# dfm/emcee

Measured on NVIDIA H100. Metric: walker-steps/sec (nwalkers x iters / s), higher is better.
Workload: dtype f64

## Files before the change

emcee_b200/csrc/dense_dmma.cu:

```cuda
#include <math.h>

#include "engine.cuh"
#include "tma.cuh"

namespace eb {

namespace {

constexpr int DMMA_CONSUMERS = 8;
constexpr int DMMA_THREADS = 64 * DMMA_CONSUMERS;
constexpr int NI = 2;
constexpr int DMMA_PRODUCER_REGS = 64;
constexpr int DMMA_CONSUMER_REGS = 192;
static_assert((DMMA_THREADS / 2) * (DMMA_PRODUCER_REGS + DMMA_CONSUMER_REGS) <= 65536, "register file of one SM");
__host__ __device__ constexpr bool dmma_rebalance(int KB, bool HAS_MEAN, bool BOUNDED) {
  return !BOUNDED && (KB >= 15 || (HAS_MEAN && KB >= 11));
}

__device__ __forceinline__ void dmma1688(double (&c)[4], double2 a01, double2 a23, double b0, double b1) {
  asm volatile(
      "mma.sync.aligned.m16n8k8.row.col.f64.f64.f64.f64 {%0,%1,%2,%3}, {%4,%5,%6,%7}, {%8,%9}, {%0,%1,%2,%3};"
      : "+d"(c[0]), "+d"(c[1]), "+d"(c[2]), "+d"(c[3])
      : "d"(a01.x), "d"(a01.y), "d"(a23.x), "d"(a23.y), "d"(b0), "d"(b1));
}

__host__ __device__ constexpr int col_pairs(int KB) { return (KB + 1) / 2; }
__host__ __device__ constexpr int factor_dmmas(int KB) { return col_pairs(KB) * (KB - col_pairs(KB) + 1); }
__host__ __device__ constexpr size_t factor_doubles(int KB) { return (size_t)factor_dmmas(KB) * 128; }
__host__ __device__ constexpr int row_stride(int KB) { return 8 * KB + 8; }

struct TileMeta {
  double factor[8];
  double log_u[8];
  double lp_old[8];
  int32_t w[8];
};

template <int KB>
struct SmemLayout {
  static constexpr size_t L_doubles = factor_doubles(KB);
  static constexpr size_t mu_doubles = 8 * KB;
  static constexpr size_t slot_doubles = 2 * 8 * row_stride(KB);
  static constexpr size_t off_mu = L_doubles;
  static constexpr size_t off_slots = off_mu + mu_doubles;
  static constexpr size_t off_meta = off_slots + DMMA_CONSUMERS * slot_doubles;
  static constexpr size_t meta_bytes = sizeof(TileMeta) * 2 * DMMA_CONSUMERS;
  static constexpr size_t off_bars_bytes = off_meta * sizeof(double) + meta_bytes;
  static constexpr int nbars = 1 + 3 * DMMA_CONSUMERS;
  static constexpr size_t off_abort_bytes = off_bars_bytes + nbars * sizeof(uint64_t);
  static constexpr size_t off_inbox_bytes = off_abort_bytes + 16;
  static constexpr size_t total_bytes = off_inbox_bytes + sizeof(int32_t) * 2 * 8 * DMMA_CONSUMERS;
};

template <int KB, bool HAS_MEAN>
__device__ __forceinline__ double tile_sumsq(const double (&q)[2 * KB], const double* sL, const double* sMu, int lane,
                                             int g, int t) {
  constexpr int NP = col_pairs(KB);
  double rs0 = 0.0, rs1 = 0.0;
  const double* aptr = sL + 2 * lane;
#pragma unroll
  for (int m0 = 0; m0 < NP; m0 += NI) {
    double c[NI][4];
#pragma unroll
    for (int n = 0; n < NI; ++n) c[n][0] = c[n][1] = c[n][2] = c[n][3] = 0.0;
#pragma unroll
    for (int j = 2 * m0; j < KB; ++j) {
      double x0 = q[2 * j + 0], x1 = q[2 * j + 1];
      if (HAS_MEAN) {
        const double2 m2 = *reinterpret_cast<const double2*>(sMu + 8 * j + 2 * t);
        x0 -= m2.x;
        x1 -= m2.y;
      }
#pragma unroll
      for (int n = 0; n < NI; ++n) {
        if (m0 + n < NP && j >= 2 * (m0 + n)) {
          const double2 a01 = *reinterpret_cast<const double2*>(aptr);
          const double2 a23 = *reinterpret_cast<const double2*>(aptr + 64);
          dmma1688(c[n], a01, a23, x0, x1);
          aptr += 128;
        }
      }
    }
#pragma unroll
    for (int n = 0; n < NI; ++n) {
      rs0 = fma(c[n][0], c[n][0], rs0);
      rs0 = fma(c[n][2], c[n][2], rs0);
      rs1 = fma(c[n][1], c[n][1], rs1);
      rs1 = fma(c[n][3], c[n][3], rs1);
    }
  }
#pragma unroll
  for (int o = 4; o < 32; o <<= 1) {
    rs0 += __shfl_xor_sync(0xffffffffu, rs0, o);
    rs1 += __shfl_xor_sync(0xffffffffu, rs1, o);
  }
  const double e = __shfl_sync(0xffffffffu, rs0, g >> 1), o = __shfl_sync(0xffffffffu, rs1, g >> 1);
  return (g & 1) ? o : e;
}

__device__ __forceinline__ bool grid_wait(const unsigned long long* counter, unsigned long long target, int* status) {
  const long long t0 = clock64();
  while (*reinterpret_cast<const volatile unsigned long long*>(counter) < target) {
    __nanosleep(32);
    if (clock64() - t0 > 60000000000ll) {
      atomicOr(status, FLAG_COMM_TIMEOUT);
      return false;
    }
  }
  __threadfence();
  return true;
}

__device__ __forceinline__ bool peer_wait(const unsigned* my_flags, int rank, int nranks, unsigned target, int lane,
                                          int* status) {
  bool ok = true;
  if (lane < nranks && lane != rank) {
    const volatile unsigned* f = my_flags + lane;
    const long long t0 = clock64();
    while ((int)(*f - target) < 0) {
      __nanosleep(64);
      if (clock64() - t0 > 60000000000ll) {
        atomicOr(status, FLAG_COMM_TIMEOUT);
        ok = false;
        break;
      }
    }
  }
  __threadfence_system();
  return __all_sync(0xffffffffu, ok);
}

template <int KB, bool HAS_MEAN, bool BOUNDED, bool TIMELINE>
__global__ void __launch_bounds__(DMMA_THREADS, 1)
    half_step_dense_dmma_kernel(const HalfStepArgs a, const HalfDesc d0, const HalfDesc* __restrict__ descs,
                                const int nhalf, unsigned long long* gbar, const unsigned long long gbar_base) {
  constexpr int D = 8 * KB;
  constexpr int RS = row_stride(KB);
  using SL = SmemLayout<KB>;
  extern __shared__ __align__(16) unsigned char smem_raw[];
  double* sL = reinterpret_cast<double*>(smem_raw);
  double* sMu = sL + SL::off_mu;
  double* sSlots = sL + SL::off_slots;
  TileMeta* sMeta = reinterpret_cast<TileMeta*>(sL + SL::off_meta);
  uint64_t* bars = reinterpret_cast<uint64_t*>(smem_raw + SL::off_bars_bytes);
  volatile int* sAbort = reinterpret_cast<volatile int*>(smem_raw + SL::off_abort_bytes);
  volatile int* sPeers = sAbort + 1;
  int32_t* sInbox = reinterpret_cast<int32_t*>(smem_raw + SL::off_inbox_bytes);
  uint64_t* barL = bars;
  uint64_t* barFull = bars + 1;
  uint64_t* barReady = bars + 1 + DMMA_CONSUMERS;
  uint64_t* barFree = bars + 1 + 2 * DMMA_CONSUMERS;

  const int tid = threadIdx.x, lane = tid & 31, warp = tid >> 5;
  const bool is_producer = warp >= DMMA_CONSUMERS;
  const int pair = is_producer ? warp - DMMA_CONSUMERS : warp;
  const int g = lane >> 2, t = lane & 3;

  if (tid == 0) {
    *sAbort = 0;
    *sPeers = 0;
    mbar_init(barL, 1);
    for (int c = 0; c < DMMA_CONSUMERS; ++c) {
      mbar_init(barFull + c, 1);
      mbar_init(barReady + c, 1);
      mbar_init(barFree + c, 1);
    }
    asm volatile("fence.mbarrier_init.release.cluster;" ::: "memory");
  }
  if (HAS_MEAN)
    for (int k = tid; k < D; k += DMMA_THREADS) sMu[k] = a.model.params[k];
  __syncthreads();

  const int tstride = (int)gridDim.x * DMMA_CONSUMERS;
  const int tile0 = (int)blockIdx.x + (int)gridDim.x * pair;
  double* slot = sSlots + (size_t)pair * SL::slot_doubles;
  double* myS = slot + (size_t)g * RS + 2 * t;
  double* myC = myS + 8 * RS;
  TileMeta* meta = sMeta + 2 * pair;
  const bool multi = a.p2p_peer_flags != nullptr;
  unsigned k = 0;

  constexpr bool REBALANCE = dmma_rebalance(KB, HAS_MEAN, BOUNDED);
  if (is_producer) {
    if constexpr (REBALANCE) asm volatile("setmaxnreg.dec.sync.aligned.u32 %0;" ::"n"(DMMA_PRODUCER_REGS));
    const long long t_entry_p = clock64();
    long long* tlp = (TIMELINE && lane == 0)
                         ? a.timeline + ((size_t)blockIdx.x * DMMA_CONSUMERS + pair) * TL_TILES * TL_EVENTS : nullptr;
    const double dm1 = (double)a.D - 1.0;
    const int row = lane & 7;
    struct Prep {
      int32_t w, wp;
      double zz, factor, log_u, lp_old;
      bool valid, remote;
    };
    for (int h = 0; h < nhalf; ++h) {
      const HalfDesc d = (h == 0) ? d0 : descs[h];
      const int32_t* order = a.order + (size_t)d.order_step * a.N;
      const int2 rg = a.range ? a.range[(size_t)d.order_step * MAX_SPLITS + d.split] : make_int2(0, d.a_count);
      const int i_lo = rg.x, i_hi = rg.y;
      const int ntiles = (int)(((int64_t)i_hi - i_lo + 7) >> 3);
      const int64_t Nc = a.N - d.a_count;
      const int32_t* aperm = a.aperm ? a.aperm + (size_t)d.order_step * a.N + d.a_start : nullptr;
      auto prep = [&](int tile, bool with_lp) -> Prep {
        Prep p;
        int i = i_lo + tile * 8 + row;
        p.valid = i < i_hi;
        if (!p.valid) i = i_hi - 1;
        if (aperm) i = __ldg(aperm + i);
        const u32x4 A = draw_words(a.seed, d.step, (uint32_t)d.split, TAG_PROP_A, (uint32_t)i);
        const double tt = __dadd_rn(__dmul_rn(__dsub_rn(a.p0, 1.0), u53(A.x, A.y)), 1.0);
        p.zz = __ddiv_rn(__dmul_rn(tt, tt), a.p0);
        const int64_t r = (int64_t)bounded64(A.z, A.w, (uint64_t)Nc);
        p.w = __ldg(order + d.a_start + i);
        p.wp = __ldg(order + (r < d.a_start ? r : r + d.a_count));
        const u32x4 U = draw_words(a.seed, d.step, (uint32_t)d.split, TAG_ACCEPT, (uint32_t)i);
        p.log_u = log(u53(U.x, U.y));
        p.factor = __dmul_rn(dm1, log(p.zz));
        p.lp_old = with_lp ? a.logp[p.w] : 0.0;
        p.remote = multi && (p.wp / a.rows_per_rank != a.p2p_rank);
        return p;
      };
      auto peers_ready = [&]() -> bool {
        if (!multi || *sPeers > h) return true;
        if (pair == 0) {
          if (!peer_wait(a.p2p_my_flags, a.p2p_rank, a.p2p_nranks, a.p2p_wait + (unsigned)h, lane, a.status)) {
            *sAbort = 1;
            return false;
          }
          __syncwarp();
          if (lane == 0) *sPeers = h + 1;
        } else {
          while (*sPeers <= h) {
            if (*sAbort) return false;
            __nanosleep(64);
          }
        }
        asm volatile("fence.proxy.async;" ::: "memory");
        return true;
      };
      auto request = [&](const Prep& p, int lo, int hi) {
        if (lane >= lo && lane < hi) {
          const bool partner = lane >= 8;
          const int32_t wr = partner ? p.wp : p.w;
          const double* base =
              (partner && a.peer_coords != nullptr) ? a.peer_coords[wr / a.rows_per_rank] : a.coords;
          bulk_g2s(slot + (size_t)(partner ? 8 : 0) * RS + (size_t)row * RS, base + (size_t)wr * D,
                   (unsigned)(D * sizeof(double)), barFull + pair);
        }
      };
      auto publish = [&](const Prep& p, int par) {
        TileMeta* m = meta + par;
        if (lane < 8) {
          m->factor[row] = p.factor;
          m->log_u[row] = p.log_u;
          m->lp_old[row] = p.lp_old;
          m->w[row] = p.valid ? p.w : -1;
        }
      };
      auto issue = [&](Prep& p, int par, bool load_lp) -> bool {
        if (__any_sync(0xffffffffu, p.remote) && !peers_ready()) return false;
        if (lane == 0) mbar_arrive_expect_tx(barFull + pair, 16u * D * (unsigned)sizeof(double));
        __syncwarp();
        request(p, 0, 16);
        if (load_lp) p.lp_old = a.logp[p.w];
        publish(p, par);
        return true;
      };
      Prep cur{}, nxt{};
      const bool early = h == 0 && a.dmma_early_own && tile0 < ntiles;
      if (early) {
        cur = prep(tile0, true);
        if (lane == 0) mbar_arrive_expect_tx(barFull + pair, 16u * D * (unsigned)sizeof(double));
        __syncwarp();
        if (tlp) tlp[6] = clock64() - t_entry_p;
        request(cur, 0, 8);
      } else if (tile0 < ntiles) {
        cur = prep(tile0, false);
      }
      if (h == 0) {
        pdl_wait();
        pdl_launch_dependents();
        if (multi && !a.aperm && !peers_ready()) return;
        if (tile0 < ntiles) {
          if (a.dmma_stagger && pair >= DMMA_CONSUMERS / 2)
            mbar_wait_for(barFull + pair - DMMA_CONSUMERS / 2, 0, multi ? 40000 : 12000);
          if (early) {
            request(cur, 8, 16);
            publish(cur, (int)(k & 1u));
          } else {
            if (tlp) tlp[6] = clock64() - t_entry_p;
            if (!issue(cur, (int)(k & 1u), true)) return;
          }
        }
        if (pair == 0 && !peers_ready()) return;
        if (tile0 + tstride < ntiles) nxt = prep(tile0 + tstride, true);
      } else {
        if (tile0 + tstride < ntiles) nxt = prep(tile0 + tstride, false);
        bool ok = true;
        if (lane == 0) ok = grid_wait(gbar, gbar_base + (unsigned long long)h * gridDim.x, a.status);
        ok = __shfl_sync(0xffffffffu, ok, 0);
        if (!ok) {
          *sAbort = 1;
          return;
        }
        asm volatile("fence.proxy.async;" ::: "memory");
        if (tile0 < ntiles) {
          if (k > 0 && !mbar_wait_abortable(barFree + pair, (k - 1) & 1u, sAbort)) return;
          if (!issue(cur, (int)(k & 1u), true)) return;
        }
      }
      for (int tile = tile0; tile < ntiles; tile += tstride, ++k) {
        const double zz = __shfl_sync(0xffffffffu, cur.zz, g);
        if (!mbar_wait_abortable(barFull + pair, k & 1u, sAbort)) return;
        long long* tlq = (tlp && h == nhalf - 1 && (tile - tile0) / tstride < TL_TILES && lane == 0)
                             ? tlp + ((tile - tile0) / tstride) * TL_EVENTS : nullptr;
        if (tlq) tlq[7] = clock64() - t_entry_p;
        if constexpr (BOUNDED) {
          bool in = true;
#pragma unroll
          for (int j = 0; j < KB; ++j) {
            const double2 s2 = *reinterpret_cast<const double2*>(myS + 8 * j);
            const double2 c2 = *reinterpret_cast<const double2*>(myC + 8 * j);
            double2 q2;
            q2.x = __dsub_rn(c2.x, __dmul_rn(__dsub_rn(c2.x, s2.x), zz));
            q2.y = __dsub_rn(c2.y, __dmul_rn(__dsub_rn(c2.y, s2.y), zz));
            *reinterpret_cast<double2*>(myC + 8 * j) = q2;
            const double2 l2 = __ldg(reinterpret_cast<const double2*>(a.model.lo + 8 * j + 2 * t));
            const double2 h2 = __ldg(reinterpret_cast<const double2*>(a.model.hi + 8 * j + 2 * t));
            in &= (l2.x <= q2.x) & (q2.x <= h2.x) & (l2.y <= q2.y) & (q2.y <= h2.y);
          }
          in &= __shfl_xor_sync(0xffffffffu, in, 1);
          in &= __shfl_xor_sync(0xffffffffu, in, 2);
          if (t == 0) sInbox[(2 * pair + (k & 1u)) * 8 + g] = in ? 1 : 0;
        } else {
#pragma unroll
          for (int j = 0; j < KB; ++j) {
            const double2 s2 = *reinterpret_cast<const double2*>(myS + 8 * j);
            const double2 c2 = *reinterpret_cast<const double2*>(myC + 8 * j);
            double2 q2;
            q2.x = __dsub_rn(c2.x, __dmul_rn(__dsub_rn(c2.x, s2.x), zz));
            q2.y = __dsub_rn(c2.y, __dmul_rn(__dsub_rn(c2.y, s2.y), zz));
            *reinterpret_cast<double2*>(myC + 8 * j) = q2;
          }
        }
        __syncwarp();
        if (lane == 0) mbar_arrive(barReady + pair);
        if (tlq) tlq[8] = clock64() - t_entry_p;
        if (tile + tstride < ntiles) {
          cur = nxt;
          if (!mbar_wait_abortable(barFree + pair, k & 1u, sAbort)) return;
          if (tlq && (tile - tile0) / tstride + 1 < TL_TILES)
            tlq[TL_EVENTS + 6] = clock64() - t_entry_p;
          if (!issue(cur, (int)((k + 1) & 1u), h > 0 && tile == tile0)) return;
          if (tile + 2 * tstride < ntiles) nxt = prep(tile + 2 * tstride, true);
        }
      }
    }
    return;
  }

  if constexpr (REBALANCE) asm volatile("setmaxnreg.inc.sync.aligned.u32 %0;" ::"n"(DMMA_CONSUMER_REGS));
  if (tid == 0) {
    constexpr unsigned bytes = (unsigned)(SL::L_doubles * sizeof(double));
    mbar_arrive_expect_tx(barL, bytes);
    bulk_g2s(sL, a.model.chol, bytes, barL);
  }
  const long long t_entry = clock64();
  long long* tl = TIMELINE ? a.timeline + ((size_t)blockIdx.x * DMMA_CONSUMERS + pair) * TL_TILES * TL_EVENTS : nullptr;
  pdl_wait();
  pdl_launch_dependents();
  bool alive = mbar_wait_abortable_notrap(barL, 0, sAbort, a.status, FLAG_WAIT_TIMEOUT);
  for (int h = 0; h < nhalf; ++h) {
    const HalfDesc d = (h == 0) ? d0 : descs[h];
    const int2 rg = a.range ? a.range[(size_t)d.order_step * MAX_SPLITS + d.split] : make_int2(0, d.a_count);
    const int ntiles = (int)(((int64_t)rg.y - rg.x + 7) >> 3);
    unsigned kk = 0;
    bool peers_passed = false;
    for (int tile = tile0; alive && tile < ntiles; tile += tstride, ++k, ++kk) {
      const TileMeta* m = meta + (k & 1u);
      long long* tlk = (tl && h == nhalf - 1 && kk < TL_TILES && lane == 0) ? tl + kk * TL_EVENTS : nullptr;
      if (tlk) {
        tlk[0] = (long long)tile;
        tlk[1] = clock64() - t_entry;
      }
      if (!mbar_wait_abortable_notrap(barReady + pair, k & 1u, sAbort, a.status, FLAG_WAIT_TIMEOUT)) {
        alive = false;
        break;
      }
      if (tlk) tlk[2] = clock64() - t_entry;
      double q[2 * KB];
#pragma unroll
      for (int j = 0; j < KB; ++j) {
        const double2 q2 = *reinterpret_cast<const double2*>(myC + 8 * j);
        q[2 * j + 0] = q2.x;
        q[2 * j + 1] = q2.y;
      }
      __syncwarp();
      if (lane == 0) mbar_arrive(barFree + pair);
      if (tlk) tlk[3] = clock64() - t_entry;

      const double rs = tile_sumsq<KB, HAS_MEAN>(q, sL, sMu, lane, g, t);
      const int32_t w = m->w[g];
      const double factor = m->factor[g], log_u = m->log_u[g], lp_old = m->lp_old[g];
      const double lp_new = (BOUNDED && sInbox[(2 * pair + (k & 1u)) * 8 + g] == 0) ? -INFINITY : -0.5 * rs;
      if (tlk) tlk[4] = clock64() - t_entry;

      if (!isfinite(lp_new)) {
        bool any_inf = false, any_nan = false;
#pragma unroll
        for (int e = 0; e < 2 * KB; ++e) {
          any_inf |= isinf(q[e]);
          any_nan |= isnan(q[e]);
        }
        if (any_inf) atomicOr(a.status, FLAG_INF_PARAM);
        if (any_nan) atomicOr(a.status, FLAG_NAN_PARAM);
        if (isnan(lp_new)) atomicOr(a.status, FLAG_NAN_LOGPROB);
      }

      const double lnpdiff = __dsub_rn(__dadd_rn(factor, lp_new), lp_old);
      const bool acc = (w >= 0) && (lnpdiff > log_u);
      if (multi && !peers_passed) {
        while (*sPeers <= h) {
          if (*sAbort) break;
          __nanosleep(64);
        }
        peers_passed = !*sAbort;
        if (!peers_passed) {
          alive = false;
          break;
        }
      }
      if (acc) {
        double* dst = a.coords + (size_t)w * D + 2 * t;
#pragma unroll
        for (int j = 0; j < KB; ++j) *reinterpret_cast<double2*>(dst + 8 * j) = make_double2(q[2 * j], q[2 * j + 1]);
      }
      if (w >= 0 && t == 0) {
        if (acc) {
          a.logp[w] = lp_new;
          atomicAdd(a.nacc + w, 1ull);
        }
        a.accepted[w] = acc ? 1 : 0;
      }
      if (tlk) tlk[5] = clock64() - t_entry;
    }
    if (h + 1 < nhalf) {
      __threadfence();
      asm volatile("bar.sync 1, %0;" ::"r"(32 * DMMA_CONSUMERS) : "memory");
      if (*sAbort) alive = false;
      if (tid == 0 && alive) {
        __threadfence();
        atomicAdd(gbar, 1ull);
      }
    }
  }
  if (multi) {
    __threadfence_system();
    asm volatile("bar.sync 1, %0;" ::"r"(32 * DMMA_CONSUMERS) : "memory");
    if (tid == 0 && !*sAbort) {
      const unsigned prev = atomicAdd(a.p2p_done, 1u);
      if (prev == gridDim.x - 1) {
        *a.p2p_done = 0;
        __threadfence_system();
        for (int r = 0; r < a.p2p_nranks; ++r)
          if (r != a.p2p_rank)
            atomicExch_system(a.p2p_peer_flags[r] + a.p2p_rank, a.p2p_signal + (unsigned)(nhalf - 1));
      }
    }
  }
}

template <int KB, bool HAS_MEAN>
__global__ void __launch_bounds__(256) logprob_dense_dmma_kernel(const ModelDev m, const double* __restrict__ x,
                                                                 const int64_t rows, double* __restrict__ out,
                                                                 int* status) {
  constexpr int D = 8 * KB;
  extern __shared__ __align__(16) unsigned char smem_raw[];
  double* sL = reinterpret_cast<double*>(smem_raw);
  double* sMu = sL + factor_doubles(KB);
  uint64_t* barL = reinterpret_cast<uint64_t*>(sMu + D);
  const int tid = threadIdx.x, lane = tid & 31, warp = tid >> 5;
  const int g = lane >> 2, t = lane & 3;
  if (tid == 0) {
    mbar_init(barL, 1);
    asm volatile("fence.mbarrier_init.release.cluster;" ::: "memory");
  }
  if (HAS_MEAN)
    for (int k = tid; k < D; k += blockDim.x) sMu[k] = m.params[k];
  __syncthreads();
  if (tid == 0) {
    constexpr unsigned bytes = (unsigned)(factor_doubles(KB) * sizeof(double));
    mbar_arrive_expect_tx(barL, bytes);
    bulk_g2s(sL, m.chol, bytes, barL);
  }
  const int64_t ntiles = (rows + 7) >> 3;
  bool waited = false;
  for (int64_t tile = (int64_t)blockIdx.x * 8 + warp; tile < ntiles; tile += (int64_t)gridDim.x * 8) {
    int64_t r = tile * 8 + g;
    const bool valid = r < rows;
    if (!valid) r = rows - 1;
    const double* src = x + (size_t)r * D + 2 * t;
    double q[2 * KB];
    bool any_inf = false, any_nan = false, in = true;
#pragma unroll
    for (int j = 0; j < KB; ++j) {
      const double2 v = __ldcg(reinterpret_cast<const double2*>(src + 8 * j));
      q[2 * j + 0] = v.x;
      q[2 * j + 1] = v.y;
      any_inf |= isinf(v.x) | isinf(v.y);
      any_nan |= isnan(v.x) | isnan(v.y);
      if (m.lo != nullptr) {
        const double2 l2 = __ldg(reinterpret_cast<const double2*>(m.lo + 8 * j + 2 * t));
        const double2 h2 = __ldg(reinterpret_cast<const double2*>(m.hi + 8 * j + 2 * t));
        in &= (l2.x <= v.x) & (v.x <= h2.x) & (l2.y <= v.y) & (v.y <= h2.y);
      }
    }
    in &= __shfl_xor_sync(0xffffffffu, in, 1);
    in &= __shfl_xor_sync(0xffffffffu, in, 2);
    if (valid && any_inf) atomicOr(status, FLAG_INF_PARAM);
    if (valid && any_nan) atomicOr(status, FLAG_NAN_PARAM);
    if (!waited) {
      mbar_wait(barL, 0);
      waited = true;
    }
    const double rs = tile_sumsq<KB, HAS_MEAN>(q, sL, sMu, lane, g, t);
    const double lp = in ? -0.5 * rs : -INFINITY;
    if (valid && t == 0) {
      out[r] = lp;
      if (isnan(lp)) atomicOr(status, FLAG_NAN_LOGPROB);
    }
  }
}

template <int KB>
cudaError_t launch_lp_t(const ModelDev& m, const double* x, int64_t rows, double* out, int* status, int sm_count,
                        cudaStream_t st) {
  const size_t smem = (factor_doubles(KB) + 8 * KB) * sizeof(double) + sizeof(uint64_t);
  const bool has_mean = m.s0 != 0.0;
  auto kern = has_mean ? logprob_dense_dmma_kernel<KB, true> : logprob_dense_dmma_kernel<KB, false>;
  if (smem > 48 * 1024) {
    cudaError_t e = cudaFuncSetAttribute(kern, cudaFuncAttributeMaxDynamicSharedMemorySize, (int)smem);
    if (e != cudaSuccess) return e;
  }
  if (rows <= 0) return cudaSuccess;
  const int64_t want = (((rows + 7) >> 3) + 7) / 8;
  const int grid = (int)(want < 2 * sm_count ? want : 2 * sm_count);
  kern<<<grid, 256, smem, st>>>(m, x, rows, out, status);
  return cudaGetLastError();
}

template <int KB>
cudaError_t launch_t(const HalfStepArgs& a, const HalfDesc& d0, const HalfDesc* descs_dev, int nhalf, int max_count,
                     unsigned long long* gbar, unsigned long long gbar_base, int sm_count, bool pdl, int* grid_out,
                     cudaStream_t st) {
  const size_t smem = SmemLayout<KB>::total_bytes;
  const bool has_mean = a.model.s0 != 0.0;
  const bool bounded = a.model.lo != nullptr;
  const bool timeline = a.timeline != nullptr;
  using Kern = decltype(&half_step_dense_dmma_kernel<KB, false, false, false>);
  static const Kern kerns[8] = {
      half_step_dense_dmma_kernel<KB, false, false, false>, half_step_dense_dmma_kernel<KB, true, false, false>,
      half_step_dense_dmma_kernel<KB, false, true, false>,  half_step_dense_dmma_kernel<KB, true, true, false>,
      half_step_dense_dmma_kernel<KB, false, false, true>,  half_step_dense_dmma_kernel<KB, true, false, true>,
      half_step_dense_dmma_kernel<KB, false, true, true>,   half_step_dense_dmma_kernel<KB, true, true, true>};
  const int variant = (has_mean ? 1 : 0) + (bounded ? 2 : 0) + (timeline ? 4 : 0);
  const Kern kern = kerns[variant];
  static bool configured[8][64] = {};
  int dev = 0;
  cudaGetDevice(&dev);
  if (dev < 0 || dev >= 64 || !configured[variant][dev]) {
    cudaError_t e = cudaFuncSetAttribute(kern, cudaFuncAttributeMaxDynamicSharedMemorySize, (int)smem);
    if (e != cudaSuccess) return e;
    if (dev >= 0 && dev < 64) configured[variant][dev] = true;
  }
  *grid_out = 0;
  if (max_count <= 0 || nhalf <= 0) return cudaSuccess;
  const int64_t ntiles = ((int64_t)max_count + 7) / 8;
  const int grid = (int)(ntiles < sm_count ? ntiles : sm_count);
  *grid_out = grid;
  HalfStepArgs args = a;
  HalfDesc first = d0;
  if (nhalf == 1) {
    cudaLaunchConfig_t cfg{};
    cfg.gridDim = dim3(grid);
    cfg.blockDim = dim3(DMMA_THREADS);
    cfg.dynamicSmemBytes = smem;
    cfg.stream = st;
    cudaLaunchAttribute attr[1];
    attr[0].id = cudaLaunchAttributeProgrammaticStreamSerialization;
    attr[0].val.programmaticStreamSerializationAllowed = 1;
    cfg.attrs = attr;
    cfg.numAttrs = pdl ? 1 : 0;
    return cudaLaunchKernelEx(&cfg, kern, args, first, descs_dev, nhalf, gbar, gbar_base);
  }
  void* params[] = {(void*)&args, (void*)&first, (void*)&descs_dev, (void*)&nhalf, (void*)&gbar, (void*)&gbar_base};
  return cudaLaunchCooperativeKernel((const void*)kern, dim3(grid), dim3(DMMA_THREADS), params, smem, st);
}

}

bool dense_dmma_supported(int D) { return D >= 8 && D <= 128 && D % 8 == 0; }

size_t dense_dmma_factor_doubles(int D) { return factor_doubles(D / 8); }

void dense_dmma_pack_factor(const double* L, int D, double* packed) {
  const int KB = D / 8, NP = col_pairs(KB);
  size_t idx = 0;
  for (int m0 = 0; m0 < NP; m0 += NI)
    for (int j = 2 * m0; j < KB; ++j)
      for (int n = 0; n < NI; ++n) {
        const int m = m0 + n;
        if (m >= NP || j < 2 * m) continue;
        for (int half = 0; half < 2; ++half)
          for (int lane = 0; lane < 32; ++lane) {
            const int g = lane >> 2, t = lane & 3, row = 8 * j + 2 * t + half;
            for (int hi = 0; hi < 2; ++hi) {
              const int col = 16 * m + 8 * hi + g;
              packed[idx++] = (col < D && col <= row) ? L[(size_t)row * D + col] : 0.0;
            }
          }
      }
}

cudaError_t launch_logprob_dense_dmma(const ModelDev& m, int D, const double* x, int64_t rows, double* out,
                                      int* status, int sm_count, cudaStream_t st) {
#define EB_LP_CASE(KB) \
  case 8 * KB:         \
    return launch_lp_t<KB>(m, x, rows, out, status, sm_count, st);
  switch (D) {
    EB_LP_CASE(1)
    EB_LP_CASE(2)
    EB_LP_CASE(3)
    EB_LP_CASE(4)
    EB_LP_CASE(5)
    EB_LP_CASE(6)
    EB_LP_CASE(7)
    EB_LP_CASE(8)
    EB_LP_CASE(9)
    EB_LP_CASE(10)
    EB_LP_CASE(11)
    EB_LP_CASE(12)
    EB_LP_CASE(13)
    EB_LP_CASE(14)
    EB_LP_CASE(15)
    EB_LP_CASE(16)
  }
#undef EB_LP_CASE
  return cudaErrorNotSupported;
}

cudaError_t launch_dense_dmma(const HalfStepArgs& a, const HalfDesc& d0, const HalfDesc* descs_dev, int nhalf,
                              int max_count, unsigned long long* gbar, unsigned long long gbar_base, int sm_count,
                              bool pdl, int* grid_out, cudaStream_t st) {
#define EB_DMMA_CASE(KB) \
  case 8 * KB:           \
    return launch_t<KB>(a, d0, descs_dev, nhalf, max_count, gbar, gbar_base, sm_count, pdl, grid_out, st);
  switch (a.D) {
    EB_DMMA_CASE(1)
    EB_DMMA_CASE(2)
    EB_DMMA_CASE(3)
    EB_DMMA_CASE(4)
    EB_DMMA_CASE(5)
    EB_DMMA_CASE(6)
    EB_DMMA_CASE(7)
    EB_DMMA_CASE(8)
    EB_DMMA_CASE(9)
    EB_DMMA_CASE(10)
    EB_DMMA_CASE(11)
    EB_DMMA_CASE(12)
    EB_DMMA_CASE(13)
    EB_DMMA_CASE(14)
    EB_DMMA_CASE(15)
    EB_DMMA_CASE(16)
  }
#undef EB_DMMA_CASE
  return cudaErrorNotSupported;
}

}
```

Before: 946.3 million.

## Move stretch-move proposal compute from producer warps into consumer warps

The producer no longer computes the proposal q = c - (c - s)*zz and the bounds check in shared memory. It publishes zz in the tile metadata and arrives on barFull, and the consumer computes q and the bounds mask straight into registers. This removes the barReady handshake, the extra shared-memory write and read of q, and the inbox. Under register rebalancing, the accept-term logs are deferred to publish time so the producer keeps fewer live registers. The register split shifts further toward the consumers, and rebalancing is now also enabled for BOUNDED at large KB. In exchange the consumer warps carry more arithmetic per tile, which can lengthen the consumer-bound critical path.

Result: faster. 971.3 million (median of 6 runs) (+2.6%).

```diff
diff --git a/emcee_b200/csrc/dense_dmma.cu b/emcee_b200/csrc/dense_dmma.cu
--- a/emcee_b200/csrc/dense_dmma.cu
+++ b/emcee_b200/csrc/dense_dmma.cu
@@ -1,4 +1,6 @@
 #include <math.h>
+
+#include <type_traits>
 
 #include "engine.cuh"
 #include "tma.cuh"
@@ -10,11 +12,11 @@
 constexpr int DMMA_CONSUMERS = 8;
 constexpr int DMMA_THREADS = 64 * DMMA_CONSUMERS;
 constexpr int NI = 2;
-constexpr int DMMA_PRODUCER_REGS = 64;
-constexpr int DMMA_CONSUMER_REGS = 192;
+constexpr int DMMA_PRODUCER_REGS = 56;
+constexpr int DMMA_CONSUMER_REGS = 200;
 static_assert((DMMA_THREADS / 2) * (DMMA_PRODUCER_REGS + DMMA_CONSUMER_REGS) <= 65536, "register file of one SM");
 __host__ __device__ constexpr bool dmma_rebalance(int KB, bool HAS_MEAN, bool BOUNDED) {
-  return !BOUNDED && (KB >= 15 || (HAS_MEAN && KB >= 11));
+  return KB >= 15 || (HAS_MEAN && !BOUNDED && KB >= 11);
 }
 
 __device__ __forceinline__ void dmma1688(double (&c)[4], double2 a01, double2 a23, double b0, double b1) {
@@ -30,6 +32,7 @@
 __host__ __device__ constexpr int row_stride(int KB) { return 8 * KB + 8; }
 
 struct TileMeta {
+  double zz[8];
   double factor[8];
   double log_u[8];
   double lp_old[8];
@@ -46,10 +49,9 @@
   static constexpr size_t off_meta = off_slots + DMMA_CONSUMERS * slot_doubles;
   static constexpr size_t meta_bytes = sizeof(TileMeta) * 2 * DMMA_CONSUMERS;
   static constexpr size_t off_bars_bytes = off_meta * sizeof(double) + meta_bytes;
-  static constexpr int nbars = 1 + 3 * DMMA_CONSUMERS;
+  static constexpr int nbars = 1 + 2 * DMMA_CONSUMERS;
   static constexpr size_t off_abort_bytes = off_bars_bytes + nbars * sizeof(uint64_t);
-  static constexpr size_t off_inbox_bytes = off_abort_bytes + 16;
-  static constexpr size_t total_bytes = off_inbox_bytes + sizeof(int32_t) * 2 * 8 * DMMA_CONSUMERS;
+  static constexpr size_t total_bytes = off_abort_bytes + 16;
 };
 
 template <int KB, bool HAS_MEAN>
@@ -145,11 +147,9 @@
   uint64_t* bars = reinterpret_cast<uint64_t*>(smem_raw + SL::off_bars_bytes);
   volatile int* sAbort = reinterpret_cast<volatile int*>(smem_raw + SL::off_abort_bytes);
   volatile int* sPeers = sAbort + 1;
-  int32_t* sInbox = reinterpret_cast<int32_t*>(smem_raw + SL::off_inbox_bytes);
   uint64_t* barL = bars;
   uint64_t* barFull = bars + 1;
-  uint64_t* barReady = bars + 1 + DMMA_CONSUMERS;
-  uint64_t* barFree = bars + 1 + 2 * DMMA_CONSUMERS;
+  uint64_t* barFree = bars + 1 + DMMA_CONSUMERS;
 
   const int tid = threadIdx.x, lane = tid & 31, warp = tid >> 5;
   const bool is_producer = warp >= DMMA_CONSUMERS;
@@ -161,8 +161,7 @@
     *sPeers = 0;
     mbar_init(barL, 1);
     for (int c = 0; c < DMMA_CONSUMERS; ++c) {
-      mbar_init(barFull + c, 1);
-      mbar_init(barReady + c, 1);
+      mbar_init(barFull + c, 2);
       mbar_init(barFree + c, 1);
     }
     asm volatile("fence.mbarrier_init.release.cluster;" ::: "memory");
@@ -188,11 +187,15 @@
                          ? a.timeline + ((size_t)blockIdx.x * DMMA_CONSUMERS + pair) * TL_TILES * TL_EVENTS : nullptr;
     const double dm1 = (double)a.D - 1.0;
     const int row = lane & 7;
-    struct Prep {
-      int32_t w, wp;
-      double zz, factor, log_u, lp_old;
+    struct PrepLean {
+      int32_t w, wp, i;
+      double zz, lp_old;
       bool valid, remote;
     };
+    struct PrepAhead : PrepLean {
+      double factor, log_u;
+    };
+    using Prep = std::conditional_t<REBALANCE, PrepLean, PrepAhead>;
     for (int h = 0; h < nhalf; ++h) {
       const HalfDesc d = (h == 0) ? d0 : descs[h];
       const int32_t* order = a.order + (size_t)d.order_step * a.N;
@@ -201,6 +204,11 @@
       const int ntiles = (int)(((int64_t)i_hi - i_lo + 7) >> 3);
       const int64_t Nc = a.N - d.a_count;
       const int32_t* aperm = a.aperm ? a.aperm + (size_t)d.order_step * a.N + d.a_start : nullptr;
+      auto accept_terms = [&](int32_t i, double zz, double* factor, double* log_u) {
+        const u32x4 U = draw_words(a.seed, d.step, (uint32_t)d.split, TAG_ACCEPT, (uint32_t)i);
+        *factor = __dmul_rn(dm1, log(zz));
+        *log_u = log(u53(U.x, U.y));
+      };
       auto prep = [&](int tile, bool with_lp) -> Prep {
         Prep p;
         int i = i_lo + tile * 8 + row;
@@ -211,11 +219,10 @@
         const double tt = __dadd_rn(__dmul_rn(__dsub_rn(a.p0, 1.0), u53(A.x, A.y)), 1.0);
         p.zz = __ddiv_rn(__dmul_rn(tt, tt), a.p0);
         const int64_t r = (int64_t)bounded64(A.z, A.w, (uint64_t)Nc);
+        p.i = i;
         p.w = __ldg(order + d.a_start + i);
         p.wp = __ldg(order + (r < d.a_start ? r : r + d.a_count));
-        const u32x4 U = draw_words(a.seed, d.step, (uint32_t)d.split, TAG_ACCEPT, (uint32_t)i);
-        p.log_u = log(u53(U.x, U.y));
-        p.factor = __dmul_rn(dm1, log(p.zz));
+        if constexpr (!REBALANCE) accept_terms(i, p.zz, &p.factor, &p.log_u);
         p.lp_old = with_lp ? a.logp[p.w] : 0.0;
         p.remote = multi && (p.wp / a.rows_per_rank != a.p2p_rank);
         return p;
@@ -251,11 +258,18 @@
       auto publish = [&](const Prep& p, int par) {
         TileMeta* m = meta + par;
         if (lane < 8) {
-          m->factor[row] = p.factor;
-          m->log_u[row] = p.log_u;
+          m->zz[row] = p.zz;
+          if constexpr (REBALANCE) {
+            accept_terms(p.i, p.zz, &m->factor[row], &m->log_u[row]);
+          } else {
+            m->factor[row] = p.factor;
+            m->log_u[row] = p.log_u;
+          }
           m->lp_old[row] = p.lp_old;
           m->w[row] = p.valid ? p.w : -1;
         }
+        __syncwarp();
+        if (lane == 0) mbar_arrive(barFull + pair);
       };
       auto issue = [&](Prep& p, int par, bool load_lp) -> bool {
         if (__any_sync(0xffffffffu, p.remote) && !peers_ready()) return false;
@@ -310,47 +324,11 @@
         }
       }
       for (int tile = tile0; tile < ntiles; tile += tstride, ++k) {
-        const double zz = __shfl_sync(0xffffffffu, cur.zz, g);
-        if (!mbar_wait_abortable(barFull + pair, k & 1u, sAbort)) return;
-        long long* tlq = (tlp && h == nhalf - 1 && (tile - tile0) / tstride < TL_TILES && lane == 0)
-                             ? tlp + ((tile - tile0) / tstride) * TL_EVENTS : nullptr;
-        if (tlq) tlq[7] = clock64() - t_entry_p;
-        if constexpr (BOUNDED) {
-          bool in = true;
-#pragma unroll
-          for (int j = 0; j < KB; ++j) {
-            const double2 s2 = *reinterpret_cast<const double2*>(myS + 8 * j);
-            const double2 c2 = *reinterpret_cast<const double2*>(myC + 8 * j);
-            double2 q2;
-            q2.x = __dsub_rn(c2.x, __dmul_rn(__dsub_rn(c2.x, s2.x), zz));
-            q2.y = __dsub_rn(c2.y, __dmul_rn(__dsub_rn(c2.y, s2.y), zz));
-            *reinterpret_cast<double2*>(myC + 8 * j) = q2;
-            const double2 l2 = __ldg(reinterpret_cast<const double2*>(a.model.lo + 8 * j + 2 * t));
-            const double2 h2 = __ldg(reinterpret_cast<const double2*>(a.model.hi + 8 * j + 2 * t));
-            in &= (l2.x <= q2.x) & (q2.x <= h2.x) & (l2.y <= q2.y) & (q2.y <= h2.y);
-          }
-          in &= __shfl_xor_sync(0xffffffffu, in, 1);
-          in &= __shfl_xor_sync(0xffffffffu, in, 2);
-          if (t == 0) sInbox[(2 * pair + (k & 1u)) * 8 + g] = in ? 1 : 0;
-        } else {
-#pragma unroll
-          for (int j = 0; j < KB; ++j) {
-            const double2 s2 = *reinterpret_cast<const double2*>(myS + 8 * j);
-            const double2 c2 = *reinterpret_cast<const double2*>(myC + 8 * j);
-            double2 q2;
-            q2.x = __dsub_rn(c2.x, __dmul_rn(__dsub_rn(c2.x, s2.x), zz));
-            q2.y = __dsub_rn(c2.y, __dmul_rn(__dsub_rn(c2.y, s2.y), zz));
-            *reinterpret_cast<double2*>(myC + 8 * j) = q2;
-          }
-        }
-        __syncwarp();
-        if (lane == 0) mbar_arrive(barReady + pair);
-        if (tlq) tlq[8] = clock64() - t_entry_p;
         if (tile + tstride < ntiles) {
           cur = nxt;
           if (!mbar_wait_abortable(barFree + pair, k & 1u, sAbort)) return;
-          if (tlq && (tile - tile0) / tstride + 1 < TL_TILES)
-            tlq[TL_EVENTS + 6] = clock64() - t_entry_p;
+          const int kk = (tile - tile0) / tstride + 1;
+          if (tlp && h == nhalf - 1 && kk < TL_TILES) tlp[kk * TL_EVENTS + 6] = clock64() - t_entry_p;
           if (!issue(cur, (int)((k + 1) & 1u), h > 0 && tile == tile0)) return;
           if (tile + 2 * tstride < ntiles) nxt = prep(tile + 2 * tstride, true);
         }
@@ -383,17 +361,29 @@
         tlk[0] = (long long)tile;
         tlk[1] = clock64() - t_entry;
       }
-      if (!mbar_wait_abortable_notrap(barReady + pair, k & 1u, sAbort, a.status, FLAG_WAIT_TIMEOUT)) {
+      if (!mbar_wait_abortable_notrap(barFull + pair, k & 1u, sAbort, a.status, FLAG_WAIT_TIMEOUT)) {
         alive = false;
         break;
       }
       if (tlk) tlk[2] = clock64() - t_entry;
+      const double zz = m->zz[g];
       double q[2 * KB];
+      bool in = true;
 #pragma unroll
       for (int j = 0; j < KB; ++j) {
-        const double2 q2 = *reinterpret_cast<const double2*>(myC + 8 * j);
-        q[2 * j + 0] = q2.x;
-        q[2 * j + 1] = q2.y;
+        const double2 s2 = *reinterpret_cast<const double2*>(myS + 8 * j);
+        const double2 c2 = *reinterpret_cast<const double2*>(myC + 8 * j);
+        q[2 * j + 0] = __dsub_rn(c2.x, __dmul_rn(__dsub_rn(c2.x, s2.x), zz));
+        q[2 * j + 1] = __dsub_rn(c2.y, __dmul_rn(__dsub_rn(c2.y, s2.y), zz));
+        if constexpr (BOUNDED) {
+          const double2 l2 = __ldg(reinterpret_cast<const double2*>(a.model.lo + 8 * j + 2 * t));
+          const double2 h2 = __ldg(reinterpret_cast<const double2*>(a.model.hi + 8 * j + 2 * t));
+          in &= (l2.x <= q[2 * j]) & (q[2 * j] <= h2.x) & (l2.y <= q[2 * j + 1]) & (q[2 * j + 1] <= h2.y);
+        }
+      }
+      if constexpr (BOUNDED) {
+        in &= __shfl_xor_sync(0xffffffffu, in, 1);
+        in &= __shfl_xor_sync(0xffffffffu, in, 2);
       }
       __syncwarp();
       if (lane == 0) mbar_arrive(barFree + pair);
@@ -402,7 +392,7 @@
       const double rs = tile_sumsq<KB, HAS_MEAN>(q, sL, sMu, lane, g, t);
       const int32_t w = m->w[g];
       const double factor = m->factor[g], log_u = m->log_u[g], lp_old = m->lp_old[g];
-      const double lp_new = (BOUNDED && sInbox[(2 * pair + (k & 1u)) * 8 + g] == 0) ? -INFINITY : -0.5 * rs;
+      const double lp_new = (BOUNDED && !in) ? -INFINITY : -0.5 * rs;
       if (tlk) tlk[4] = clock64() - t_entry;
 
       if (!isfinite(lp_new)) {
```
